# Iselix/kwiiyatta

Measured on AMD Instinct MI355X. Metric: frames/sec end-to-end analyse->align->convert->synth, 48 kHz 5 ms hop, higher is better.
Workload: dtype f64; 1 GPU; config3: 48 kHz source (10 s, T=2001) + target (11 s, T=2201) pairs: CheapTrick+D4C of both, pad with freshly drawn silent spectra, sp2mc, FastDTW(radius 32) align, GMM(64 comp, D=144)+MLPG convert, mc2sp, WORLD synthesis; pairs_per_gpu=32, streams_per_gpu=4, GPU_MAX_HW_QUEUES=4, launch=the whole step is one captured HIP graph, gmm_model_prepared=once per converter (the per-mixture matrices depend on the GMM only), parallelism=pairs in lockstep x32 per GPU, pair-per-GPU x1, no collective

## Files before the change

### kwiiyatta_amd/csrc/kwy_d4c.hip

```cpp
#include <math.h>

#include <vector>

#include "kwy_internal.hpp"

#define D4C_SAFE 0.000000000001
#define D4C_FLOOR_F0 47.0
#define D4C_FREQ_INTERVAL 3000.0
#define D4C_UPPER_LIMIT 15000.0
#define D4C_MAX_BANDS 8

enum { D4C_HANNING = 1, D4C_BLACKMAN = 2 };

__device__ __forceinline__ double d4c_window(int type, int i, int half, double ratio, int fs, double cf0) {
  const double c1 = kwy_cos_pi_range(KWY_PI * ((2.0 * (i - half) / ratio) / fs) * cf0);
  return type == D4C_HANNING ? 0.5 * c1 + 0.5 : 0.42 + 0.5 * c1 + 0.08 * (2.0 * c1 * c1 - 1.0);
}

struct d4c_window_walk {
  double c, s, cd, sd;
  __device__ __forceinline__ d4c_window_walk(int i0, int step, int half, double ratio, int fs, double cf0) {
    kwy_sincos_pi_range(KWY_PI * ((2.0 * (i0 - half) / ratio) / fs) * cf0, &s, &c);
    sincos(KWY_PI * ((2.0 * step / ratio) / fs) * cf0, &sd, &cd);
  }
// ... 316 lines not shown
__device__ inline void d4c_subtract_smoothed(double *io, double *S, double *tot, double width, int fs, int N, int kmax) {
  const int H = N / 2;
  int boundary = (int)(width * N / fs) + 1;
  if (boundary > H / 2) boundary = H / 2;
  const int L = min(H + boundary * 2 + 1, kmax + boundary * 2 + 4);
  kwy_block_cumsum_of<NT, D4C_SMOOTH_CHUNK>([&](int i) {
    double m;
    if (i < boundary) m = io[boundary - i];
    else if (i < H + boundary) m = io[i - boundary];
    else m = io[H - (i - (H + boundary))];
    return m * fs / N;
  }, S, L, tot);
  const double origin = -(boundary - 0.5) * fs / N;
  const double inv_dfi = (double)N / fs, inv_width = 1.0 / width;
  const d4c_taps taps = d4c_smoothing_taps(origin, inv_dfi, width);
  for (int k = threadIdx.x; k <= min(H, kmax); k += NT) io[k] = io[k] - d4c_smoothed_bin(S, L, taps, k) * inv_width;
  __syncthreads();
}

template <int NT, int RK>
__device__ inline void d4c_linear_smoothing_regs(const double *in, double (&outv)[RK], double *S, double *tot,
                                                 double width, int fs, int N) {
  const int H = N / 2;
  int boundary = (int)(width * N / fs) + 1;
  if (boundary > H / 2) boundary = H / 2;
  const int L = H + boundary * 2 + 1;
  kwy_block_cumsum_of<NT, D4C_SMOOTH_CHUNK>([&](int i) {
    double m;
    if (i < boundary) m = in[boundary - i];
    else if (i < H + boundary) m = in[i - boundary];
    else m = in[H - (i - (H + boundary))];
    return m * fs / N;
  }, S, L, tot);
  const double origin = -(boundary - 0.5) * fs / N;
  const double inv_dfi = (double)N / fs, inv_width = 1.0 / width;
  const d4c_taps taps = d4c_smoothing_taps(origin, inv_dfi, width);
#pragma unroll
  for (int r = 0; r < RK; ++r) {
    const int k = threadIdx.x + NT * r;
    outv[r] = 0.0;
    if (k <= H) outv[r] = fmax(d4c_smoothed_bin(S, L, taps, k) * inv_width, 0.0);
  }
  __syncthreads();
}

__device__ __forceinline__ kwy_c d4c_opaque(kwy_c v) {
  asm volatile("" : "+v"(v.x), "+v"(v.y));
  return v;
}

template <int LOG2N>
struct d4c_nt { static constexpr int value = LOG2N >= 13 ? 512 : 256; };
template <int LOG2N>
static constexpr size_t d4c_body_lds() {
  constexpr int N = 1 << LOG2N, H = N / 2, NT = d4c_nt<LOG2N>::value;
  return sizeof(double) * (NT + 16 + D4C_MAX_BANDS + 2) + sizeof(uint32_t) * KWY_EBASE_WORDS +
         (LOG2N >= 12 ? 0 : 8192) + sizeof(double) * ((H + 2) + (2 * H + 2) + 2) +
         ((sizeof(uint32_t) * KWY_SELECT_WORDS(NT) > sizeof(double) * (2 * H + 4))
              ? sizeof(uint32_t) * KWY_SELECT_WORDS(NT) - sizeof(double) * (2 * H + 4) : 0);
}

template <int LOG2N>
__global__ __launch_bounds__(d4c_nt<LOG2N>::value, LOG2N >= 13 ? 1 : 3) void k_d4c_body(
    d4c_batch batch, d4c_params p, kwy_randn_src rs,
    const uint4 *__restrict__ poly, const kwy_c *__restrict__ twH, const kwy_c *__restrict__ twN,
    long long *__restrict__ dbg) {
  constexpr int N = 1 << LOG2N, H = N / 2;
  constexpr int NT = d4c_nt<LOG2N>::value;
  constexpr int E = N / NT;
  constexpr int RK = (H + 1 + NT - 1) / NT;
  constexpr int HEX = 16 * NT / N;
  static_assert(HEX >= 1, "workgroup narrower than N/16");
#define D4C_STAMP(n) do { if (dbg && threadIdx.x == 0 && blockIdx.x == (unsigned)dbg[63]) dbg[n] = clock64(); } while (0)
  extern __shared__ double smem[];
  double *tot = smem;
  double *red = tot + NT;
  double *coarse = red + 16;
  uint32_t *e = (uint32_t *)(coarse + D4C_MAX_BANDS + 2);
  double *jt_own = (double *)(e + KWY_EBASE_WORDS);
  double *A0 = jt_own + (LOG2N >= 12 ? 0 : 1024);
  kwy_c *B = (kwy_c *)(A0 + (H + 2));
  double *Bd = (double *)B;
  double *P = A0, *Dv = A0;
  double *S = Bd;
  uint4 *jtab = (uint4 *)((LOG2N >= 12) ? A0 : jt_own);

  const int tid = threadIdx.x;
  const int utt = batch.find(blockIdx.x);
  const int64_t frame = (int)blockIdx.x - batch.start[utt];
  const double *__restrict__ x = batch.u[utt].x;
  const int x_length = batch.u[utt].x_length;
  const uint64_t *__restrict__ offs3 = batch.u[utt].offs3;
  const uint64_t *__restrict__ draws_before = batch.u[utt].offs_lt + batch.u[utt].T;
  double *__restrict__ dvbuf = batch.u[utt].dvbuf;
  const double f0v = kwy_uniform(batch.u[utt].f0[frame]);
  double *o = batch.u[utt].out + frame * p.K;
  if (f0v == 0.0 || kwy_uniform(batch.u[utt].ap0[frame]) <= p.threshold) {
    for (int k = tid; k < p.K; k += NT) o[k] = 1.0 - D4C_SAFE;
    return;
  }
  const double cf0 = kwy_uniform(f0v > D4C_FLOOR_F0 ? f0v : D4C_FLOOR_F0);
  const double pos = kwy_uniform(batch.u[utt].tpos[frame]);

  D4C_STAMP(0);
  kwy_c tw4[4];
  kwy_fft_thread_twiddles<LOG2N - 1, NT>(twH, tw4);
  const kwy_c twb = twN[tid];
  const uint64_t dbase = *draws_before;
  const uint64_t dpos0 = dbase + offs3[3 * frame], dpos1 = dbase + offs3[3 * frame + 1], dpos2 = dbase + offs3[3 * frame + 2];
  const bool cache = dpos2 + (uint64_t)(2 * kwy_matlab_round(4.0 * p.fs / cf0 / 2.0) + 1) <= rs.n;

  D4C_STAMP(1);
  constexpr int RP = (H / 2 + NT - 1) / NT;
  double cen_lo[RP], cen_hi[RP];
  double *mid = coarse;
  {
    double av[E];
    for (int which = 0; which < 2; ++which) {
      const int tid = kwy_tid_opaque();
      double cpos = which == 0 ? pos - 0.25 / cf0 : pos + 0.25 / cf0;
      d4c_frame_window<N, NT>(x, x_length, p, cf0, cpos, D4C_BLACKMAN, which == 0 ? dpos0 : dpos1, rs, poly, e, jtab, Bd, true, red, av,
                              A0, cache ? 1 + which : 0);
      __syncthreads();
      if (!(tid & 1)) {
#pragma unroll
        for (int r = 0; r < E; ++r) { const int i = tid + NT * r; Bd[i] = av[r]; Bd[i + 1] = av[r] * (i + 1.0); }
      }
      __syncthreads();
      D4C_STAMP(2 + which * 2);
      kwy_fft_inplace_w<LOG2N - 1, NT, false>(B, tw4);
      kwy_c Ek[RP], Eh[RP];
#pragma unroll
      for (int r = 0; r < RP; ++r) {
        const int pp = tid + NT * r;
        Ek[r] = Eh[r] = kwy_c{0.0, 0.0};
        if (pp < H / 2) { Ek[r] = B[pp]; Eh[r] = B[(H - pp) & (H - 1)]; }
      }
      if (tid == 0) { mid[0] = B[H / 2].x; mid[1] = B[H / 2].y; }
      __syncthreads();
      if (tid & 1) {
#pragma unroll
        for (int r = 0; r < E; ++r) { const int i = tid + NT * r; Bd[i - 1] = av[r]; Bd[i] = av[r] * (i + 1.0); }
      }
      __syncthreads();
      kwy_fft_inplace_w<LOG2N - 1, NT, false>(B, tw4);
#pragma unroll
      for (int r = 0; r < RP; ++r) {
        const int pp = tid + NT * r;
        if (pp < H / 2) {
          const kwy_c w = kwy_tw_hex(d4c_opaque(twb), HEX * r);
          const kwy_c Ok = B[pp], Oh = B[(H - pp) & (H - 1)];
          const kwy_c t = cmulf(w, Ok);
          const kwy_c u = cmulf(kwy_c{-w.x, w.y}, Oh);
          const kwy_c zp = cadd(Ek[r], t), zhp = csub(Ek[r], t);
          const kwy_c zq = cadd(Eh[r], u), znp = csub(Eh[r], u);
          const double lo = 2.0 * __builtin_fma(zp.x, znp.y, zp.y * znp.x);
          const double hi = 2.0 * __builtin_fma(zq.x, zhp.y, zq.y * zhp.x);
          cen_lo[r] = which == 0 ? lo : cen_lo[r] + lo;
          cen_hi[r] = which == 0 ? hi : cen_hi[r] + hi;
        }
      }
      if (tid == 0) {
        const kwy_c Em = {mid[0], mid[1]}, Om = B[H / 2];
        const kwy_c t = {Om.y, -Om.x};
        const kwy_c za = cadd(Em, t), zb = csub(Em, t);
        const double v = 2.0 * __builtin_fma(za.x, zb.y, za.y * zb.x);
        mid[2] = which == 0 ? v : mid[2] + v;
      }
      __syncthreads();
      D4C_STAMP(3 + which * 2);
    }

    D4C_STAMP(6);
    d4c_frame_window<N, NT>(x, x_length, p, cf0, pos, D4C_HANNING, dpos2, rs, poly, e, jtab, Bd, false, red, av, A0, cache ? 2 : 0);
#pragma unroll
    for (int r = 0; r < E; ++r) Bd[tid + NT * r] = av[r];
    __syncthreads();
  }
  D4C_STAMP(7);
  kwy_fft_inplace_w<LOG2N - 1, NT, false>(B, tw4);
  D4C_STAMP(8);
  double pv[RK];
  {
    constexpr int Q = (H / 2) / NT;
    static_assert(RK == 2 * Q + 1, "pairs per thread");
#pragma unroll
    for (int q = 0; q < Q; ++q)
      kwy_rfft_pair_power2_w<LOG2N - 1>(B, tid + NT * q, kwy_tw_hex(d4c_opaque(twb), HEX * q), &pv[2 * q], &pv[2 * q + 1]);
    pv[2 * Q] = 0.0;
    if (tid == 0) {
      double pm;
      kwy_rfft_pair_power2_w<LOG2N - 1>(B, H / 2, kwy_c{0.0, -1.0}, &pv[2 * Q], &pm);
    }
    __syncthreads();
#pragma unroll
    for (int q = 0; q < Q; ++q) {
      const int k = tid + NT * q;
      P[k] = pv[2 * q];
      P[H - k] = pv[2 * q + 1];
    }
    if (tid == 0) P[H / 2] = pv[2 * Q];
  }
  __syncthreads();
  d4c_dc_correction<NT>(P, S, cf0, p.fs, N);
  d4c_linear_smoothing_regs<NT, RK>(P, pv, S, tot, cf0, p.fs, N);

  D4C_STAMP(9);
#pragma unroll
  for (int r = 0; r < RP; ++r) {
    const int pp = tid + NT * r;
    if (pp < H / 2) { Dv[pp] = cen_lo[r]; Dv[H - pp] = cen_hi[r]; }
  }
  if (tid == 0) Dv[H / 2] = mid[2];
  __syncthreads();
  d4c_dc_correction<NT>(Dv, S, cf0, p.fs, N);
#pragma unroll
  for (int r = 0; r < RK; ++r)
    if (tid + NT * r <= H) Dv[tid + NT * r] = Dv[tid + NT * r] / pv[r];
  __syncthreads();
  const int kdv = p.dv_len - 1;
  d4c_linear_smoothing<NT>(Dv, Dv, S, tot, cf0 / 2.0, p.fs, N, kdv + 2 * ((int)(cf0 * N / p.fs) + 1) + 4);
  d4c_subtract_smoothed<NT>(Dv, S, tot, cf0, p.fs, N, kdv);

  D4C_STAMP(10);
  {
    double *dv = dvbuf + (size_t)frame * p.dv_stride;
    for (int k = tid; k < p.dv_len; k += NT) dv[k] = Dv[k];
  }
  D4C_STAMP(15);
#undef D4C_STAMP
}

template <int LOG2N>
static constexpr size_t d4c_bands_lds() {
  constexpr int N = 1 << LOG2N, H = N / 2, NT = d4c_nt<LOG2N>::value;
  return sizeof(double) * (16 + D4C_MAX_BANDS + 2 + 2 * NT) + sizeof(double) * ((2 * H + 2) + 2) +
         ((sizeof(uint32_t) * KWY_SELECT_WORDS(NT) > sizeof(double) * (2 * H + 4))
              ? sizeof(uint32_t) * KWY_SELECT_WORDS(NT) - sizeof(double) * (2 * H + 4) : 0);
}

template <int LOG2N, bool SPARSE>
__global__ __launch_bounds__(d4c_nt<LOG2N>::value, LOG2N >= 13 ? 2 : 4) void k_d4c_bands(
    d4c_batch batch, d4c_params p, const kwy_c *__restrict__ twH,
    const kwy_c *__restrict__ twN, const double *__restrict__ nuttall, long long *__restrict__ dbg) {
  constexpr int N = 1 << LOG2N, H = N / 2;
  constexpr int NT = d4c_nt<LOG2N>::value;
  constexpr int E = N / NT;
  constexpr int RK = (H + 1 + NT - 1) / NT;
  constexpr int HEX = 16 * NT / N;
#define D4C_STAMP(n) do { if (dbg && threadIdx.x == 0 && blockIdx.x == (unsigned)dbg[63]) dbg[n] = clock64(); } while (0)
  extern __shared__ double smem[];
  double *red = smem;
  double *coarse = red + 16;
  double *wns = coarse + D4C_MAX_BANDS + 2;
  kwy_c *B = (kwy_c *)(wns + 2 * NT);
  double *Bd = (double *)B;
  uint32_t *hist = (uint32_t *)B;

  const int tid = threadIdx.x;
  const int utt = batch.find(blockIdx.x);
  const int64_t frame = (int)blockIdx.x - batch.start[utt];
  const double *__restrict__ dvbuf = batch.u[utt].dvbuf;
  double *__restrict__ out = batch.u[utt].out;
  const double f0v = kwy_uniform(batch.u[utt].f0[frame]);
  if (f0v == 0.0 || kwy_uniform(batch.u[utt].ap0[frame]) <= p.threshold) return;
  const double cf0 = kwy_uniform(f0v > D4C_FLOOR_F0 ? f0v : D4C_FLOOR_F0);
  const double *Dv = dvbuf + (size_t)frame * p.dv_stride;
  D4C_STAMP(16);

  const int boundary = __builtin_amdgcn_readfirstlane(kwy_matlab_round(N * 8.0 / p.window_length));
  const int half_window_length = p.window_length / 2;
  constexpr bool sparse = SPARSE;
  double ns0 = 0.0, ns1 = 0.0, ns2 = 0.0, nutr[4] = {0.0, 0.0, 0.0, 0.0};
  if constexpr (sparse) {
    if (2 * tid < p.window_length) ns0 = nuttall[2 * tid];
    if (2 * tid + 1 < p.window_length) ns1 = nuttall[2 * tid + 1];
    wns[2 * tid] = ns0; wns[2 * tid + 1] = ns1;
  } else {
#pragma unroll
    for (int r = 0; r < 4; ++r)
      if (tid + NT * r < p.window_length) nutr[r] = nuttall[tid + NT * r];
  }
  const bool mine0 = sparse && tid < H / 8 && 2 * tid < p.window_length;
  const bool mine1 = sparse && tid < H / 8 && 2 * tid + 1 < p.window_length;
  const double *Dfirst = Dv + ((int)(D4C_FREQ_INTERVAL * N / p.fs) - half_window_length);
  double nx0 = (mine0 && p.nbands > 0) ? Dfirst[2 * tid] : 0.0;
  double nx1 = (mine1 && p.nbands > 0) ? Dfirst[2 * tid + 1] : 0.0;
  for (int b = 0; b < p.nbands; ++b) {
    const int tid = kwy_tid_opaque();
    kwy_c tw4[4];
    kwy_fft_thread_twiddles<LOG2N - 1, NT>(twH + (tid - (int)threadIdx.x), tw4);
    const kwy_c twb = twN[tid];
    const double *Dc = Dv + ((int)(D4C_FREQ_INTERVAL * (b + 1) * N / p.fs) - half_window_length);
    const double c0 = nx0, c1 = nx1;
    if (b == 1) D4C_STAMP(17);
    {
      const double *Dn = Dv + ((int)(D4C_FREQ_INTERVAL * (b + 2) * N / p.fs) - half_window_length);
      const bool more = b + 1 < p.nbands;
      nx0 = (mine0 && more) ? Dn[2 * tid] : 0.0;
      nx1 = (mine1 && more) ? Dn[2 * tid + 1] : 0.0;
    }
    if constexpr (sparse) {
      kwy_c a0 = {c0 * wns[2 * tid], c1 * wns[2 * tid + 1]}, a1 = {0.0, 0.0};
      if (tid == 0 && 2 * (H / 8) < p.window_length) a1.x = Dc[2 * (H / 8)] * nuttall[2 * (H / 8)];
      kwy_fft_pass8_first_sparse_core<LOG2N - 1, NT, false>(B, kwy_tw_reg{tw4[0]}, a0, a1);
      kwy_fft_inplace_rest_w<LOG2N - 1, NT, false>(B, tw4);
      if (b == 1) D4C_STAMP(18);
    } else {
#pragma unroll
      for (int r = 0; r < E; ++r) {
        const int j = tid + NT * r;
        Bd[j] = (r < 4 && j < p.window_length) ? Dc[j] * nutr[r < 4 ? r : 0] : 0.0;
      }
      __syncthreads();
      kwy_fft_inplace_w<LOG2N - 1, NT, false>(B, tw4);
    }
    unsigned long long key[RK];
    constexpr int Q = (H / 2) / NT;
    static_assert(RK == 2 * Q + 1, "pairs per thread");
#pragma unroll
    for (int q = 0; q < Q; ++q) {
      double pk, pm;
      kwy_rfft_pair_power2_w<LOG2N - 1>(B, tid + NT * q, kwy_tw_hex(d4c_opaque(twb), HEX * q), &pk, &pm);
      key[2 * q] = (unsigned long long)__double_as_longlong(pk);
      key[2 * q + 1] = (unsigned long long)__double_as_longlong(pm);
    }
    key[2 * Q] = ~0ull;
    if (tid == 0) {
      double pk, pm;
      kwy_rfft_pair_power2_w<LOG2N - 1>(B, H / 2, kwy_c{0.0, -1.0}, &pk, &pm);
      key[2 * Q] = (unsigned long long)__double_as_longlong(pk);
    }
    __syncthreads();
    if (b == 1) D4C_STAMP(19);
    double nsmall, nall;
    kwy_block_smallest_sum<RK, NT>(key, H + 1, H - boundary, hist, red, &nsmall, &nall);
    if (b == 1) D4C_STAMP(20);
    if (dbg && tid == 0 && blockIdx.x == (unsigned)dbg[63])
      for (int q = 0; q < 12; ++q) dbg[24 + 12 * (b & 1) + q] = hist[2 * KWY_SELECT_BINS + q];
    if (tid == 0) {
      double cv = 10 * log10(nsmall / nall);
      cv = cv + (cf0 - 100) / 50.0;
      coarse[b + 1] = cv < 0.0 ? cv : 0.0;
    }
    __syncthreads();
  }
  D4C_STAMP(21);
  if (tid == 0) {
    coarse[0] = -60.0;
    coarse[p.nbands + 1] = -D4C_SAFE;
  }
  __syncthreads();
  double *o = out + frame * p.K;
  const int nn = p.nbands + 2;
  for (int k = tid; k < p.K; k += NT) {
    double xi = (double)k * p.fs / p.fft_size;
    int seg = min((int)(xi / D4C_FREQ_INTERVAL) + 1, p.nbands + 1);
    if (seg < 1) seg = 1;
    if (seg > nn - 1) seg = nn - 1;
    double xa = (seg - 1 <= p.nbands) ? (seg - 1) * D4C_FREQ_INTERVAL : p.fs / 2.0;
    double xb = (seg <= p.nbands) ? seg * D4C_FREQ_INTERVAL : p.fs / 2.0;
    double sfrac = (xi - xa) / (xb - xa);
    double v = coarse[seg - 1] + sfrac * (coarse[seg] - coarse[seg - 1]);
    o[k] = exp10(v / 20.0);
  }
  D4C_STAMP(22);
#undef D4C_STAMP
}

template <int LOG2N>
static int launch_lt(kwy_ctx *ctx, const d4c_batch &b, int fs) {
  constexpr int N = 1 << LOG2N, H = N / 2;
  const kwy_c *twH, *twN;
  const uint4 *poly;
  KWY_TRY(kwy_get_twiddles(ctx, LOG2N - 1, &twH));
  KWY_TRY(kwy_get_twiddles(ctx, LOG2N, &twN));
  constexpr int NT = d4c_nt<LOG2N>::value;
  KWY_TRY(kwy_get_poly_multi(ctx, N / NT, NT, &poly));
  size_t lds = sizeof(kwy_c) * (H + 1) + sizeof(double) * 8 + sizeof(uint32_t) * KWY_EBASE_WORDS;
  KWY_HIP(hipFuncSetAttribute((const void *)k_d4c_lovetrain<LOG2N, NT>,
                              hipFuncAttributeMaxDynamicSharedMemorySize, (int)lds));
  KWY_PROF(ctx, "k_d4c_lovetrain", hipLaunchKernelGGL((k_d4c_lovetrain<LOG2N, NT>), dim3((unsigned)b.start[b.n]), dim3(NT), lds,
                     ctx->stream, b, fs, kwy_randn(ctx), poly, twH, twN));
  KWY_HIP(hipGetLastError());
  return KWY_OK;
}
// ... 208 lines not shown
```

### kwiiyatta_amd/csrc/kwy_device.hpp

```cpp
#pragma once

#include <hip/hip_runtime.h>
#include <stdint.h>

#define KWY_THREADS 256
#define KWY_WAVES (KWY_THREADS / 64)
#define KWY_PI 3.1415926535897932384

struct kwy_rng {
  uint32_t x, y, z, w;
};

__device__ __forceinline__ void kwy_rng_seed(kwy_rng &r) {
  r.x = 123456789u; r.y = 362436069u; r.z = 521288629u; r.w = 88675123u;
}

__device__ __forceinline__ uint32_t kwy_rng_step(kwy_rng &r) {
  uint32_t t = r.x ^ (r.x << 11);
  r.x = r.y; r.y = r.z; r.z = r.w;
  r.w = (r.w ^ (r.w >> 19)) ^ (t ^ (t >> 8));
  return r.w;
}

__device__ __forceinline__ uint32_t kwy_rng_randn_raw(kwy_rng &r) {
  uint32_t tmp = kwy_rng_step(r) >> 4;
#pragma unroll
  for (int i = 0; i < 11; ++i) tmp += kwy_rng_step(r) >> 4;
  return tmp;
}
__device__ __forceinline__ double kwy_rng_randn(kwy_rng &r) {
  return kwy_rng_randn_raw(r) / 268435456.0 - 6.0;
}

__device__ __forceinline__ uint32_t kwy_wave_xor_u32(uint32_t v) {
  v ^= (uint32_t)__builtin_amdgcn_update_dpp(0, (int)v, 0x111, 0xf, 0xf, true);
  v ^= (uint32_t)__builtin_amdgcn_update_dpp(0, (int)v, 0x112, 0xf, 0xf, true);
  v ^= (uint32_t)__builtin_amdgcn_update_dpp(0, (int)v, 0x114, 0xf, 0xf, true);
  v ^= (uint32_t)__builtin_amdgcn_update_dpp(0, (int)v, 0x118, 0xf, 0xf, true);
  return (uint32_t)__builtin_amdgcn_readlane((int)v, 15) ^ (uint32_t)__builtin_amdgcn_readlane((int)v, 31) ^
         (uint32_t)__builtin_amdgcn_readlane((int)v, 47) ^ (uint32_t)__builtin_amdgcn_readlane((int)v, 63);
}

__device__ inline void kwy_wave_jump(uint32_t (&s)[4], uint64_t steps, const uint4 *__restrict__ pow2) {
  const int lane = threadIdx.x & 63;
  for (int k = 0; steps != 0; ++k, steps >>= 1) {
    if (!(steps & 1)) continue;
    const uint32_t wlo = lane < 32 ? s[0] : s[1];
    const uint32_t whi = lane < 32 ? s[2] : s[3];
    uint32_t o0 = 0, o1 = 0, o2 = 0, o3 = 0;
    uint32_t m = 0u - ((wlo >> (lane & 31)) & 1u);
    uint4 c = pow2[k * 128 + lane];
    o0 ^= c.x & m; o1 ^= c.y & m; o2 ^= c.z & m; o3 ^= c.w & m;
    m = 0u - ((whi >> (lane & 31)) & 1u);
    c = pow2[k * 128 + 64 + lane];
    o0 ^= c.x & m; o1 ^= c.y & m; o2 ^= c.z & m; o3 ^= c.w & m;
    s[0] = kwy_wave_xor_u32(o0); s[1] = kwy_wave_xor_u32(o1);
    s[2] = kwy_wave_xor_u32(o2); s[3] = kwy_wave_xor_u32(o3);
  }
}

#define KWY_EBASE_WORDS 132
__device__ inline void kwy_rng_ebase(kwy_rng s, uint32_t *e) {
  e[0] = s.x; e[1] = s.y; e[2] = s.z; e[3] = s.w;
  for (int i = 4; i < 131; ++i) e[i] = kwy_rng_step(s);
  e[131] = 0;
}

__device__ __forceinline__ void kwy_rng_combine_word(kwy_rng &r, const uint32_t *e, uint32_t bits,
                                                      uint32_t &w0, uint32_t &w1, uint32_t &w2) {
#pragma unroll 8
  for (int b = 0; b < 32; ++b) {
    uint32_t w3 = e[b + 3];
    uint32_t m = 0u - ((bits >> b) & 1u);
    r.x ^= w0 & m; r.y ^= w1 & m; r.z ^= w2 & m; r.w ^= w3 & m;
    w0 = w1; w1 = w2; w2 = w3;
  }
}

__device__ __forceinline__ kwy_rng kwy_rng_combine(const uint32_t *e, uint4 c) {
  kwy_rng r = {0, 0, 0, 0};
  uint32_t w0 = e[0], w1 = e[1], w2 = e[2];
  kwy_rng_combine_word(r, e, c.x, w0, w1, w2);
  kwy_rng_combine_word(r, e + 32, c.y, w0, w1, w2);
  kwy_rng_combine_word(r, e + 64, c.z, w0, w1, w2);
  kwy_rng_combine_word(r, e + 96, c.w, w0, w1, w2);
  return r;
}

__device__ __forceinline__ void kwy_lds_barrier() {
  asm volatile("s_waitcnt lgkmcnt(0)\n\ts_barrier" ::: "memory");
}

struct kwy_randn_src {
  const uint32_t *tab;
  uint64_t n;
  const uint4 *pow2;
};
// ... 718 lines not shown
  if constexpr (LOG2H == 12) kwy_fft_pass8<LOG2H, 9, NT, INV>(z, tw);
  if constexpr (LOG2H == 11) kwy_fft_tail<LOG2H, 2, NT, INV>(z);
  if constexpr (LOG2H == 10) kwy_fft_tail<LOG2H, 1, NT, INV>(z);
}

template <int LOG2H, int TAIL, int NT, bool INV>
__device__ __forceinline__ void kwy_fft_tail(kwy_c *z) {
  constexpr int H = 1 << LOG2H, R = 1 << TAIL, Q = H / R;
  constexpr int IT = (Q + NT - 1) / NT;
  kwy_c a[IT][R];
  const int tid = kwy_tid_opaque();
#pragma unroll
  for (int it = 0; it < IT; ++it) {
    const int j = tid + it * NT;
    if (j < Q) {
#pragma unroll
      for (int m = 0; m < R; ++m) a[it][m] = z[j + m * Q];
      if constexpr (TAIL == 2) {
        kwy_c apc = cadd(a[it][0], a[it][2]), amc = csub(a[it][0], a[it][2]);
        kwy_c bpd = cadd(a[it][1], a[it][3]), jb = kwy_rot90<INV>(csub(a[it][1], a[it][3]));
        a[it][0] = cadd(apc, bpd); a[it][1] = cadd(amc, jb);
        a[it][2] = csub(apc, bpd); a[it][3] = csub(amc, jb);
      } else {
        kwy_c s0 = cadd(a[it][0], a[it][1]), s1 = csub(a[it][0], a[it][1]);
        a[it][0] = s0; a[it][1] = s1;
      }
#pragma unroll
      for (int m = 0; m < R; ++m) z[j + m * Q] = a[it][m];
    }
  }
  __syncthreads();
}

template <int LOG2H, int NT, bool INV>
__device__ inline void kwy_fft_inplace(kwy_c *z, const kwy_c *__restrict__ tw) {
  static_assert(LOG2H >= 8 && LOG2H <= 12, "unsupported in-place FFT length");
  kwy_fft_pass8<LOG2H, 0, NT, INV>(z, tw);
  kwy_fft_pass8<LOG2H, 3, NT, INV>(z, tw);
  if constexpr (LOG2H >= 9) kwy_fft_pass8<LOG2H, 6, NT, INV>(z, tw);
  if constexpr (LOG2H == 12) kwy_fft_pass8<LOG2H, 9, NT, INV>(z, tw);
  if constexpr (LOG2H % 3 != 0) kwy_fft_tail<LOG2H, LOG2H % 3, NT, INV>(z);
}

template <int LOG2H, int NT>
__device__ __forceinline__ void kwy_fft_thread_twiddles(const kwy_c *__restrict__ twH, kwy_c (&w)[4]) {
  static_assert((1 << LOG2H) / 8 <= NT, "one butterfly per thread and pass");
  const int j = threadIdx.x;
#pragma unroll
  for (int p = 0; p < 4; ++p) {
    const int ps = (j >> (3 * p)) << (3 * p);
    w[p] = (3 * p + 3 < LOG2H + 0 && ps < (1 << LOG2H) / 8) ? twH[ps] : kwy_c{1.0, 0.0};
  }
}
template <int LOG2H, int NT, bool INV>
__device__ inline void kwy_fft_inplace_rest_w(kwy_c *z, const kwy_c (&w)[4]) {
  kwy_fft_pass8_core<LOG2H, 3, NT, INV>(z, kwy_tw_reg{w[1]});
  if constexpr (LOG2H >= 9) kwy_fft_pass8_core<LOG2H, 6, NT, INV>(z, kwy_tw_reg{w[2]});
  if constexpr (LOG2H == 12) kwy_fft_pass8_core<LOG2H, 9, NT, INV>(z, kwy_tw_reg{w[3]});
  if constexpr (LOG2H % 3 != 0) kwy_fft_tail<LOG2H, LOG2H % 3, NT, INV>(z);
}
template <int LOG2H, int NT, bool INV>
__device__ inline void kwy_fft_inplace_w(kwy_c *z, const kwy_c (&w)[4]) {
  static_assert(LOG2H >= 8 && LOG2H <= 12, "unsupported in-place FFT length");
  kwy_fft_pass8_core<LOG2H, 0, NT, INV>(z, kwy_tw_reg{w[0]});
  kwy_fft_inplace_rest_w<LOG2H, NT, INV>(z, w);
}

__device__ __forceinline__ kwy_c kwy_tw_hex(kwy_c b, int idx16) {
  if (!(idx16 & 1)) return kwy_tw_octant(b, idx16 >> 1);
  const double c1 = 0.92387953251128675613, s1 = 0.38268343236508977173;
  double wr, wi;
  switch (idx16 & 15) {
    case 1: wr = c1; wi = -s1; break;
    case 3: wr = s1; wi = -c1; break;
    case 5: wr = -s1; wi = -c1; break;
    case 7: wr = -c1; wi = -s1; break;
    case 9: wr = -c1; wi = s1; break;
    case 11: wr = -s1; wi = c1; break;
    case 13: wr = s1; wi = c1; break;
    default: wr = c1; wi = s1; break;
  }
  return {__builtin_fma(b.x, wr, -(b.y * wi)), __builtin_fma(b.x, wi, b.y * wr)};
}

template <int LOG2H, int NT>
__device__ inline void kwy_rfft_inplace(kwy_c *z, const kwy_c *__restrict__ tw, kwy_c twb,
                                   const kwy_c *__restrict__ twN = nullptr) {
  constexpr int H = 1 << LOG2H, N = 2 * H;
  constexpr int OCT = 8 * NT / N;
  kwy_fft_inplace<LOG2H, NT, false>(z, tw);
  const int tid = kwy_tid_opaque();
#pragma unroll
  for (int r = 0; r * NT <= H / 2; ++r) {
    const int k = tid + NT * r;
    if (k > H / 2) continue;
    if (k == 0) {
      const kwy_c z0 = z[0];
      z[0] = {z0.x + z0.y, 0.0};
      z[H] = {z0.x - z0.y, 0.0};
    } else {
      const kwy_c w = (OCT >= 1) ? kwy_tw_octant(twb, OCT * r) : twN[k];
      const kwy_c A = z[k], Bc = z[H - k];
      const double er = 0.5 * (A.x + Bc.x), ei = 0.5 * (A.y - Bc.y);
      const double dr = 0.5 * (A.x - Bc.x), di = 0.5 * (A.y + Bc.y);
      const double orr = di, oi = -dr;
      const double pr = __builtin_fma(orr, w.x, -(oi * w.y)), pi = __builtin_fma(orr, w.y, oi * w.x);
      z[k] = {er + pr, ei + pi};
      if (k != H - k) z[H - k] = {er - pr, -(ei - pi)};
    }
  }
  __syncthreads();
}

template <int LOG2H, int NT>
__device__ inline void kwy_irfft_inplace(kwy_c *z, const kwy_c *__restrict__ tw, kwy_c twb,
                                   const kwy_c *__restrict__ twN = nullptr) {
  constexpr int H = 1 << LOG2H, N = 2 * H;
  constexpr int OCT = 8 * NT / N;
// ... 10 lines not shown
      const kwy_c w = (OCT >= 1) ? kwy_tw_octant(twb, OCT * r) : twN[k];
      const kwy_c A = z[k], Bc = z[H - k];
      const double er = A.x + Bc.x, ei = A.y - Bc.y;
      const double dr = A.x - Bc.x, di = A.y + Bc.y;
      const double wr = w.x, wi = -w.y;
      const double orr = __builtin_fma(dr, wr, -(di * wi)), oi = __builtin_fma(dr, wi, di * wr);
      z[k] = {er - oi, ei + orr};
      if (k != H - k) z[H - k] = {er + oi, -(ei - orr)};
    }
  }
  __syncthreads();
  kwy_fft_inplace<LOG2H, NT, true>(z, tw);
}

template <int LOG2H>
__device__ __forceinline__ kwy_c kwy_rfft_bin_w(const kwy_c *z, int k, kwy_c w) {
  constexpr int H = 1 << LOG2H;
  if (k == 0) return {z[0].x + z[0].y, 0.0};
  if (k == H) return {z[0].x - z[0].y, 0.0};
  const kwy_c A = z[k];
  const kwy_c B = {z[H - k].x, -z[H - k].y};
  const double er = 0.5 * (A.x + B.x), ei = 0.5 * (A.y + B.y);
  const double dr = 0.5 * (A.x - B.x), di = 0.5 * (A.y - B.y);
  const double orr = di, oi = -dr;
  return {er + (orr * w.x - oi * w.y), ei + (orr * w.y + oi * w.x)};
}
template <int LOG2H>
__device__ __forceinline__ kwy_c kwy_rfft_bin2_w(const kwy_c *z, int k, kwy_c w) {
  constexpr int H = 1 << LOG2H;
  if (k == 0) return {2.0 * (z[0].x + z[0].y), 0.0};
  if (k == H) return {2.0 * (z[0].x - z[0].y), 0.0};
  const kwy_c A = z[k];
  const kwy_c B = {z[H - k].x, -z[H - k].y};
  const double er = A.x + B.x, ei = A.y + B.y;
  const double dr = A.x - B.x, di = A.y - B.y;
  return {__builtin_fma(dr, w.y, __builtin_fma(di, w.x, er)), __builtin_fma(-dr, w.x, __builtin_fma(di, w.y, ei))};
}
template <int LOG2H>
__device__ __forceinline__ void kwy_rfft_pair_power2_w(const kwy_c *z, int k, kwy_c w, double *pk, double *pm) {
  constexpr int H = 1 << LOG2H;
  if (k == 0) {
    const double a = 2.0 * (z[0].x + z[0].y), b = 2.0 * (z[0].x - z[0].y);
    *pk = a * a; *pm = b * b;
    return;
  }
  const kwy_c A = z[k], Bz = z[H - k];
  const double er = A.x + Bz.x, ei = A.y - Bz.y;
  const double dr = A.x - Bz.x, di = A.y + Bz.y;
  const double pr = __builtin_fma(dr, w.y, di * w.x), pi = __builtin_fma(-dr, w.x, di * w.y);
  const double xr = er + pr, xi = ei + pi, yr = er - pr, yi = ei - pi;
  *pk = __builtin_fma(xr, xr, xi * xi);
  *pm = __builtin_fma(yr, yr, yi * yi);
}
template <int LOG2H>
__device__ __forceinline__ kwy_c kwy_rfft_bin(const kwy_c *z, int k, const kwy_c *__restrict__ twN) {
  return kwy_rfft_bin_w<LOG2H>(z, k, twN[k & ((2 << LOG2H) - 1)]);
}

__device__ __forceinline__ int kwy_matlab_round(double x) {
  return x > 0 ? (int)(x + 0.5) : (int)(x - 0.5);
}
```

### kwiiyatta_amd/csrc/kwy_selftest.h

```cpp
#ifndef KWY_SELFTEST_H_
#define KWY_SELFTEST_H_
#ifdef __cplusplus
extern "C" {
#endif
int kwy_debug_smallest_sum_dev(void *stream, const double *values, int problems, int n, int m, double *out);
int kwy_debug_devmath_dev(void *stream, const double *x, int n, double *log_out, double *sin_out, double *cos_out);
#ifdef __cplusplus
}
#endif
#endif
```

### kwiiyatta_amd/csrc/selftest/kwy_selftest.hip

```cpp
#include <hip/hip_runtime.h>

#include <stdint.h>

#include "../kwy_device.hpp"
#include "../kwy_selftest.h"

#define D4C_NT 256

__global__ __launch_bounds__(D4C_NT) void k_select_selftest(const double *__restrict__ v, int n, int m,
                                                           double *__restrict__ out) {
  constexpr int RK = 9;
  __shared__ __attribute__((aligned(16))) uint32_t hist[KWY_SELECT_WORDS(D4C_NT)];
  __shared__ double red[2 * D4C_NT / 64];
  const int tid = threadIdx.x;
  const double *x = v + (size_t)blockIdx.x * n;
  unsigned long long key[RK];
#pragma unroll
  for (int r = 0; r < RK; ++r) {
    const int k = tid + D4C_NT * r;
    key[r] = k < n ? (unsigned long long)__double_as_longlong(x[k]) : ~0ull;
  }
  double s_small, s_all;
  kwy_block_smallest_sum<RK, D4C_NT>(key, n, m, hist, red, &s_small, &s_all);
  if (tid == 0) { out[2 * blockIdx.x] = s_small; out[2 * blockIdx.x + 1] = s_all; }
}

extern "C" int kwy_debug_smallest_sum_dev(void *stream, const double *values, int problems, int n, int m,
                                          double *out) {
  if (!values || !out || problems <= 0 || n <= 0 || n > 9 * D4C_NT || m <= 0 || m > n) return -1;
  hipLaunchKernelGGL(k_select_selftest, dim3(problems), dim3(D4C_NT), 0, (hipStream_t)stream, values, n, m, out);
  return hipGetLastError() == hipSuccess ? 0 : -2;
}

__global__ void k_devmath_selftest(const double *__restrict__ x, int n, double *__restrict__ lg, double *__restrict__ sn,
                                   double *__restrict__ cs) {
  const int i = blockIdx.x * blockDim.x + threadIdx.x;
  if (i >= n) return;
  lg[i] = kwy_log(x[i]);
  kwy_sincos_medium(x[i], &sn[i], &cs[i]);
}

extern "C" int kwy_debug_devmath_dev(void *stream, const double *x, int n, double *log_out, double *sin_out,
                                     double *cos_out) {
  if (!x || !log_out || !sin_out || !cos_out || n <= 0) return -1;
  hipLaunchKernelGGL(k_devmath_selftest, dim3((n + 255) / 256), dim3(256), 0, (hipStream_t)stream, x, n, log_out,
                     sin_out, cos_out);
  return hipGetLastError() == hipSuccess ? 0 : -2;
}
```

Before: 2.601 million frames/s.

## Fuse radix-4 FFT tail into register drain for 4096-point D4C transforms

```diff
diff --git a/kwiiyatta_amd/csrc/kwy_d4c.hip b/kwiiyatta_amd/csrc/kwy_d4c.hip
--- a/kwiiyatta_amd/csrc/kwy_d4c.hip
+++ b/kwiiyatta_amd/csrc/kwy_d4c.hip
@@ -392,6 +392,9 @@
 template <int LOG2N>
 struct d4c_nt { static constexpr int value = LOG2N >= 13 ? 512 : 256; };
 template <int LOG2N>
+struct d4c_drain { static constexpr bool value = LOG2N == 12; };
+#define D4C_DRAIN_TWC(twN, NT, tid) (twN)[((NT) - (tid)) & ((NT) - 1)]
+template <int LOG2N>
 static constexpr size_t d4c_body_lds() {
   constexpr int N = 1 << LOG2N, H = N / 2, NT = d4c_nt<LOG2N>::value;
   return sizeof(double) * (NT + 16 + D4C_MAX_BANDS + 2) + sizeof(uint32_t) * KWY_EBASE_WORDS +
@@ -411,6 +414,7 @@
   constexpr int RK = (H + 1 + NT - 1) / NT;
   constexpr int HEX = 16 * NT / N;
   static_assert(HEX >= 1, "workgroup narrower than N/16");
+  constexpr bool DRAIN = d4c_drain<LOG2N>::value;
 #define D4C_STAMP(n) do { if (dbg && threadIdx.x == 0 && blockIdx.x == (unsigned)dbg[63]) dbg[n] = clock64(); } while (0)
   extern __shared__ double smem[];
   double *tot = smem;
@@ -445,6 +449,8 @@
   D4C_STAMP(0);
   kwy_c tw4[4];
   kwy_fft_thread_twiddles<LOG2N - 1, NT>(twH, tw4);
+#define D4C_BODY_TW4() do { if constexpr (DRAIN) { const int ot = kwy_tid_opaque(); \
+    kwy_fft_thread_twiddles<LOG2N - 1, NT>(twH + (ot - (int)threadIdx.x), tw4); } } while (0)
   const kwy_c twb = twN[tid];
   const uint64_t dbase = *draws_before;
   const uint64_t dpos0 = dbase + offs3[3 * frame], dpos1 = dbase + offs3[3 * frame + 1], dpos2 = dbase + offs3[3 * frame + 2];
@@ -468,28 +474,51 @@
       }
       __syncthreads();
       D4C_STAMP(2 + which * 2);
-      kwy_fft_inplace_w<LOG2N - 1, NT, false>(B, tw4);
+      D4C_BODY_TW4();
+      kwy_fft_inplace_w<LOG2N - 1, NT, false, !DRAIN>(B, tw4);
       kwy_c Ek[RP], Eh[RP];
+      if constexpr (DRAIN) {
+        static_assert(RP == 4, "four pairs per thread");
+        kwy_c Em;
+        kwy_fft_tail4_drain<LOG2N - 1, NT, false>(B, Ek, Eh, Em);
+        if (tid == 0) { mid[0] = Em.x; mid[1] = Em.y; }
+      } else {
+#pragma unroll
+        for (int r = 0; r < RP; ++r) {
+          const int pp = tid + NT * r;
+          Ek[r] = Eh[r] = kwy_c{0.0, 0.0};
+          if (pp < H / 2) { Ek[r] = B[pp]; Eh[r] = B[(H - pp) & (H - 1)]; }
+        }
+        if (tid == 0) { mid[0] = B[H / 2].x; mid[1] = B[H / 2].y; }
+      }
+      __syncthreads();
+      if (tid & 1) {
+#pragma unroll
+        for (int r = 0; r < E; ++r) { const int i = tid + NT * r; Bd[i - 1] = av[r]; Bd[i] = av[r] * (i + 1.0); }
+      }
+      __syncthreads();
+      D4C_BODY_TW4();
+      kwy_fft_inplace_w<LOG2N - 1, NT, false, !DRAIN>(B, tw4);
+      kwy_c Od[DRAIN ? 4 : 1], Odh[DRAIN ? 4 : 1], twa = {0.0, 0.0}, twc = {0.0, 0.0};
+      if constexpr (DRAIN) {
+        kwy_c Om;
+        kwy_fft_tail4_drain<LOG2N - 1, NT, false>(B, Od, Odh, Om);
+        if (tid == 0) { mid[3] = Om.x; mid[4] = Om.y; }
+        twa = twN[tid];
+        twc = D4C_DRAIN_TWC(twN, NT, tid);
+      }
 #pragma unroll
       for (int r = 0; r < RP; ++r) {
         const int pp = tid + NT * r;
-        Ek[r] = Eh[r] = kwy_c{0.0, 0.0};
-        if (pp < H / 2) { Ek[r] = B[pp]; Eh[r] = B[(H - pp) & (H - 1)]; }
-      }
-      if (tid == 0) { mid[0] = B[H / 2].x; mid[1] = B[H / 2].y; }
-      __syncthreads();
-      if (tid & 1) {
-#pragma unroll
-        for (int r = 0; r < E; ++r) { const int i = tid + NT * r; Bd[i - 1] = av[r]; Bd[i] = av[r] * (i + 1.0); }
-      }
-      __syncthreads();
-      kwy_fft_inplace_w<LOG2N - 1, NT, false>(B, tw4);
-#pragma unroll
-      for (int r = 0; r < RP; ++r) {
-        const int pp = tid + NT * r;
-        if (pp < H / 2) {
-          const kwy_c w = kwy_tw_hex(d4c_opaque(twb), HEX * r);
-          const kwy_c Ok = B[pp], Oh = B[(H - pp) & (H - 1)];
+        if (DRAIN || pp < H / 2) {
+          kwy_c w, Ok, Oh;
+          if constexpr (DRAIN) {
+            w = kwy_drain_tw<LOG2N - 1, NT>(r, twa, twc);
+            Ok = Od[r]; Oh = Odh[r];
+          } else {
+            w = kwy_tw_hex(d4c_opaque(twb), HEX * r);
+            Ok = B[pp]; Oh = B[(H - pp) & (H - 1)];
+          }
           const kwy_c t = cmulf(w, Ok);
           const kwy_c u = cmulf(kwy_c{-w.x, w.y}, Oh);
           const kwy_c zp = cadd(Ek[r], t), zhp = csub(Ek[r], t);
@@ -501,7 +530,7 @@
         }
       }
       if (tid == 0) {
-        const kwy_c Em = {mid[0], mid[1]}, Om = B[H / 2];
+        const kwy_c Em = {mid[0], mid[1]}, Om = DRAIN ? kwy_c{mid[3], mid[4]} : B[H / 2];
         const kwy_c t = {Om.y, -Om.x};
         const kwy_c za = cadd(Em, t), zb = csub(Em, t);
         const double v = 2.0 * __builtin_fma(za.x, zb.y, za.y * zb.x);
@@ -518,10 +547,35 @@
     __syncthreads();
   }
   D4C_STAMP(7);
-  kwy_fft_inplace_w<LOG2N - 1, NT, false>(B, tw4);
+  D4C_BODY_TW4();
+  kwy_fft_inplace_w<LOG2N - 1, NT, false, !DRAIN>(B, tw4);
   D4C_STAMP(8);
   double pv[RK];
-  {
+  if constexpr (DRAIN) {
+    static_assert(RK == 9, "four pairs per thread and the self-paired bin");
+    const int tid = kwy_tid_opaque();
+    kwy_c lo[4], hi[4], md;
+    kwy_fft_tail4_drain<LOG2N - 1, NT, false>(B, lo, hi, md);
+    const kwy_c twa = twN[tid], twc = D4C_DRAIN_TWC(twN, NT, tid);
+#pragma unroll
+    for (int s = 0; s < 4; ++s) {
+      if (s == 0 && tid == 0) kwy_rfft_pair_power2_dc(lo[0], &pv[0], &pv[1]);
+      else kwy_rfft_pair_power2_v(lo[s], hi[s], kwy_drain_tw<LOG2N - 1, NT>(s, twa, twc), &pv[2 * s], &pv[2 * s + 1]);
+    }
+    pv[8] = 0.0;
+    if (tid == 0) {
+      double pm;
+      kwy_rfft_pair_power2_v(md, md, kwy_c{0.0, -1.0}, &pv[8], &pm);
+    }
+    __syncthreads();
+#pragma unroll
+    for (int s = 0; s < 4; ++s) {
+      const int k = kwy_drain_bin<LOG2N - 1>(s, tid);
+      P[k] = pv[2 * s];
+      P[H - k] = pv[2 * s + 1];
+    }
+    if (tid == 0) P[H / 2] = pv[8];
+  } else {
     constexpr int Q = (H / 2) / NT;
     static_assert(RK == 2 * Q + 1, "pairs per thread");
 #pragma unroll
@@ -548,7 +602,7 @@
   D4C_STAMP(9);
 #pragma unroll
   for (int r = 0; r < RP; ++r) {
-    const int pp = tid + NT * r;
+    const int pp = DRAIN ? kwy_drain_bin<LOG2N - 1>(r, tid) : tid + NT * r;
     if (pp < H / 2) { Dv[pp] = cen_lo[r]; Dv[H - pp] = cen_hi[r]; }
   }
   if (tid == 0) Dv[H / 2] = mid[2];
@@ -569,6 +623,7 @@
   }
   D4C_STAMP(15);
 #undef D4C_STAMP
+#undef D4C_BODY_TW4
 }
 
 template <int LOG2N>
@@ -588,6 +643,7 @@
   constexpr int E = N / NT;
   constexpr int RK = (H + 1 + NT - 1) / NT;
   constexpr int HEX = 16 * NT / N;
+  constexpr bool DRAIN = d4c_drain<LOG2N>::value;
 #define D4C_STAMP(n) do { if (dbg && threadIdx.x == 0 && blockIdx.x == (unsigned)dbg[63]) dbg[n] = clock64(); } while (0)
   extern __shared__ double smem[];
   double *red = smem;
@@ -644,7 +700,7 @@
       kwy_c a0 = {c0 * wns[2 * tid], c1 * wns[2 * tid + 1]}, a1 = {0.0, 0.0};
       if (tid == 0 && 2 * (H / 8) < p.window_length) a1.x = Dc[2 * (H / 8)] * nuttall[2 * (H / 8)];
       kwy_fft_pass8_first_sparse_core<LOG2N - 1, NT, false>(B, kwy_tw_reg{tw4[0]}, a0, a1);
-      kwy_fft_inplace_rest_w<LOG2N - 1, NT, false>(B, tw4);
+      kwy_fft_inplace_rest_w<LOG2N - 1, NT, false, !DRAIN>(B, tw4);
       if (b == 1) D4C_STAMP(18);
     } else {
 #pragma unroll
@@ -653,25 +709,56 @@
         Bd[j] = (r < 4 && j < p.window_length) ? Dc[j] * nutr[r < 4 ? r : 0] : 0.0;
       }
       __syncthreads();
-      kwy_fft_inplace_w<LOG2N - 1, NT, false>(B, tw4);
+      kwy_fft_inplace_w<LOG2N - 1, NT, false, !DRAIN>(B, tw4);
     }
     unsigned long long key[RK];
     constexpr int Q = (H / 2) / NT;
     static_assert(RK == 2 * Q + 1, "pairs per thread");
-#pragma unroll
-    for (int q = 0; q < Q; ++q) {
-      double pk, pm;
-      kwy_rfft_pair_power2_w<LOG2N - 1>(B, tid + NT * q, kwy_tw_hex(d4c_opaque(twb), HEX * q), &pk, &pm);
-      key[2 * q] = (unsigned long long)__double_as_longlong(pk);
-      key[2 * q + 1] = (unsigned long long)__double_as_longlong(pm);
-    }
-    key[2 * Q] = ~0ull;
-    if (tid == 0) {
-      double pk, pm;
-      kwy_rfft_pair_power2_w<LOG2N - 1>(B, H / 2, kwy_c{0.0, -1.0}, &pk, &pm);
-      key[2 * Q] = (unsigned long long)__double_as_longlong(pk);
-    }
-    __syncthreads();
+    if constexpr (DRAIN) {
+      static_assert(Q == 4 && sizeof(uint32_t) * KWY_SELECT_WORDS(NT) <= sizeof(kwy_c) * NT, "exchange clear of the histogram");
+      kwy_c lo[4], hi[4], md;
+      kwy_fft_tail4_drain<LOG2N - 1, NT, false>(B, lo, hi, md);
+      const kwy_c twc = D4C_DRAIN_TWC(twN, NT, tid);
+      double pw[8];
+#pragma unroll
+      for (int s = 0; s < 4; ++s) {
+        if (s == 0 && tid == 0) kwy_rfft_pair_power2_dc(lo[0], &pw[0], &pw[1]);
+        else kwy_rfft_pair_power2_v(lo[s], hi[s], kwy_drain_tw<LOG2N - 1, NT>(s, d4c_opaque(twb), twc), &pw[2 * s], &pw[2 * s + 1]);
+      }
+      key[2 * Q] = ~0ull;
+      if (tid == 0) {
+        double pk, pm;
+        kwy_rfft_pair_power2_v(md, md, kwy_c{0.0, -1.0}, &pk, &pm);
+        key[2 * Q] = (unsigned long long)__double_as_longlong(pk);
+      } else {
+        B[2 * NT - tid] = kwy_c{pw[4], pw[5]};
+        B[4 * NT - tid] = kwy_c{pw[6], pw[7]};
+      }
+      __syncthreads();
+      if (tid != 0) {
+        const kwy_c v1 = B[NT + tid], v3 = B[3 * NT + tid];
+        pw[4] = v1.x; pw[5] = v1.y; pw[6] = v3.x; pw[7] = v3.y;
+      }
+      key[0] = (unsigned long long)__double_as_longlong(pw[0]); key[1] = (unsigned long long)__double_as_longlong(pw[1]);
+      key[2] = (unsigned long long)__double_as_longlong(pw[4]); key[3] = (unsigned long long)__double_as_longlong(pw[5]);
+      key[4] = (unsigned long long)__double_as_longlong(pw[2]); key[5] = (unsigned long long)__double_as_longlong(pw[3]);
+      key[6] = (unsigned long long)__double_as_longlong(pw[6]); key[7] = (unsigned long long)__double_as_longlong(pw[7]);
+    } else {
+#pragma unroll
+      for (int q = 0; q < Q; ++q) {
+        double pk, pm;
+        kwy_rfft_pair_power2_w<LOG2N - 1>(B, tid + NT * q, kwy_tw_hex(d4c_opaque(twb), HEX * q), &pk, &pm);
+        key[2 * q] = (unsigned long long)__double_as_longlong(pk);
+        key[2 * q + 1] = (unsigned long long)__double_as_longlong(pm);
+      }
+      key[2 * Q] = ~0ull;
+      if (tid == 0) {
+        double pk, pm;
+        kwy_rfft_pair_power2_w<LOG2N - 1>(B, H / 2, kwy_c{0.0, -1.0}, &pk, &pm);
+        key[2 * Q] = (unsigned long long)__double_as_longlong(pk);
+      }
+      __syncthreads();
+    }
     if (b == 1) D4C_STAMP(19);
     double nsmall, nall;
     kwy_block_smallest_sum<RK, NT>(key, H + 1, H - boundary, hist, red, &nsmall, &nall);
diff --git a/kwiiyatta_amd/csrc/kwy_device.hpp b/kwiiyatta_amd/csrc/kwy_device.hpp
--- a/kwiiyatta_amd/csrc/kwy_device.hpp
+++ b/kwiiyatta_amd/csrc/kwy_device.hpp
@@ -42,7 +42,8 @@
 }
 
 __device__ inline void kwy_wave_jump(uint32_t (&s)[4], uint64_t steps, const uint4 *__restrict__ pow2) {
-  const int lane = threadIdx.x & 63;
+  int lane = threadIdx.x & 63;
+  asm volatile("" : "+v"(lane));
   for (int k = 0; steps != 0; ++k, steps >>= 1) {
     if (!(steps & 1)) continue;
     const uint32_t wlo = lane < 32 ? s[0] : s[1];
@@ -867,18 +868,18 @@
     w[p] = (3 * p + 3 < LOG2H + 0 && ps < (1 << LOG2H) / 8) ? twH[ps] : kwy_c{1.0, 0.0};
   }
 }
-template <int LOG2H, int NT, bool INV>
+template <int LOG2H, int NT, bool INV, bool TAIL = true>
 __device__ inline void kwy_fft_inplace_rest_w(kwy_c *z, const kwy_c (&w)[4]) {
   kwy_fft_pass8_core<LOG2H, 3, NT, INV>(z, kwy_tw_reg{w[1]});
   if constexpr (LOG2H >= 9) kwy_fft_pass8_core<LOG2H, 6, NT, INV>(z, kwy_tw_reg{w[2]});
   if constexpr (LOG2H == 12) kwy_fft_pass8_core<LOG2H, 9, NT, INV>(z, kwy_tw_reg{w[3]});
-  if constexpr (LOG2H % 3 != 0) kwy_fft_tail<LOG2H, LOG2H % 3, NT, INV>(z);
-}
-template <int LOG2H, int NT, bool INV>
+  if constexpr (TAIL && LOG2H % 3 != 0) kwy_fft_tail<LOG2H, LOG2H % 3, NT, INV>(z);
+}
+template <int LOG2H, int NT, bool INV, bool TAIL = true>
 __device__ inline void kwy_fft_inplace_w(kwy_c *z, const kwy_c (&w)[4]) {
   static_assert(LOG2H >= 8 && LOG2H <= 12, "unsupported in-place FFT length");
   kwy_fft_pass8_core<LOG2H, 0, NT, INV>(z, kwy_tw_reg{w[0]});
-  kwy_fft_inplace_rest_w<LOG2H, NT, INV>(z, w);
+  kwy_fft_inplace_rest_w<LOG2H, NT, INV, TAIL>(z, w);
 }
 
 __device__ __forceinline__ kwy_c kwy_tw_hex(kwy_c b, int idx16) {
@@ -995,6 +996,73 @@
   *pk = __builtin_fma(xr, xr, xi * xi);
   *pm = __builtin_fma(yr, yr, yi * yi);
 }
+__device__ __forceinline__ kwy_c kwy_rfft_bin2_v(kwy_c A, kwy_c Bz, kwy_c w) {
+  const kwy_c B = {Bz.x, -Bz.y};
+  const double er = A.x + B.x, ei = A.y + B.y;
+  const double dr = A.x - B.x, di = A.y - B.y;
+  return {__builtin_fma(dr, w.y, __builtin_fma(di, w.x, er)), __builtin_fma(-dr, w.x, __builtin_fma(di, w.y, ei))};
+}
+__device__ __forceinline__ void kwy_rfft_pair_power2_v(kwy_c A, kwy_c Bz, kwy_c w, double *pk, double *pm) {
+  const double er = A.x + Bz.x, ei = A.y - Bz.y;
+  const double dr = A.x - Bz.x, di = A.y + Bz.y;
+  const double pr = __builtin_fma(dr, w.y, di * w.x), pi = __builtin_fma(-dr, w.x, di * w.y);
+  const double xr = er + pr, xi = ei + pi, yr = er - pr, yi = ei - pi;
+  *pk = __builtin_fma(xr, xr, xi * xi);
+  *pm = __builtin_fma(yr, yr, yi * yi);
+}
+__device__ __forceinline__ void kwy_rfft_pair_power2_dc(kwy_c Z0, double *pk, double *pm) {
+  const double a = 2.0 * (Z0.x + Z0.y), b = 2.0 * (Z0.x - Z0.y);
+  *pk = a * a; *pm = b * b;
+}
+
+template <int LOG2H, int NT, bool INV>
+__device__ __forceinline__ void kwy_fft_tail4_drain(const kwy_c *z, kwy_c (&lo)[4], kwy_c (&hi)[4], kwy_c &mid) {
+  constexpr int H = 1 << LOG2H, Q = H / 4;
+  static_assert(LOG2H % 3 == 2 && NT == Q / 2, "radix-4 tail, two butterflies per thread");
+  const int t = kwy_tid_opaque();
+  const int jb = t ? Q - t : Q / 2;
+  kwy_c a[4], b[4];
+#pragma unroll
+  for (int m = 0; m < 4; ++m) { a[m] = z[t + m * Q]; b[m] = z[jb + m * Q]; }
+  {
+    const kwy_c apc = cadd(a[0], a[2]), amc = csub(a[0], a[2]);
+    const kwy_c bpd = cadd(a[1], a[3]), jq = kwy_rot90<INV>(csub(a[1], a[3]));
+    a[0] = cadd(apc, bpd); a[1] = cadd(amc, jq); a[2] = csub(apc, bpd); a[3] = csub(amc, jq);
+  }
+  {
+    const kwy_c apc = cadd(b[0], b[2]), amc = csub(b[0], b[2]);
+    const kwy_c bpd = cadd(b[1], b[3]), jq = kwy_rot90<INV>(csub(b[1], b[3]));
+    b[0] = cadd(apc, bpd); b[1] = cadd(amc, jq); b[2] = csub(apc, bpd); b[3] = csub(amc, jq);
+  }
+  const bool t0 = t == 0;
+  lo[0] = a[0]; hi[0] = t0 ? a[0] : b[3];
+  lo[1] = a[1]; hi[1] = t0 ? a[3] : b[2];
+  lo[2] = b[0]; hi[2] = t0 ? b[3] : a[3];
+  lo[3] = b[1]; hi[3] = t0 ? b[2] : a[2];
+  mid = a[2];
+}
+template <int LOG2H>
+__device__ __forceinline__ int kwy_drain_bin(int s, int t) {
+  constexpr int Q = (1 << LOG2H) / 4;
+  switch (s) {
+    case 0: return t;
+    case 1: return Q + t;
+    case 2: return t ? Q - t : Q / 2;
+    default: return t ? 2 * Q - t : Q + Q / 2;
+  }
+}
+template <int LOG2H, int NT>
+__device__ __forceinline__ kwy_c kwy_drain_tw(int s, kwy_c twa, kwy_c twc) {
+  constexpr int HEX = 16 * NT / (2 << LOG2H);
+  static_assert(HEX >= 1, "workgroup narrower than N/16");
+  switch (s) {
+    case 0: return kwy_tw_hex(twa, 0);
+    case 1: return kwy_tw_hex(twa, 2 * HEX);
+    case 2: return kwy_tw_hex(twc, HEX);
+    default: return kwy_tw_hex(twc, 3 * HEX);
+  }
+}
+
 template <int LOG2H>
 __device__ __forceinline__ kwy_c kwy_rfft_bin(const kwy_c *z, int k, const kwy_c *__restrict__ twN) {
   return kwy_rfft_bin_w<LOG2H>(z, k, twN[k & ((2 << LOG2H) - 1)]);
diff --git a/kwiiyatta_amd/csrc/kwy_selftest.h b/kwiiyatta_amd/csrc/kwy_selftest.h
--- a/kwiiyatta_amd/csrc/kwy_selftest.h
+++ b/kwiiyatta_amd/csrc/kwy_selftest.h
@@ -5,6 +5,7 @@
 #endif
 int kwy_debug_smallest_sum_dev(void *stream, const double *values, int problems, int n, int m, double *out);
 int kwy_debug_devmath_dev(void *stream, const double *x, int n, double *log_out, double *sin_out, double *cos_out);
+int kwy_debug_rfft_paths_dev(void *stream, const double *x, int problems, int log2n, double *out_old, double *out_new);
 #ifdef __cplusplus
 }
 #endif
diff --git a/kwiiyatta_amd/csrc/selftest/kwy_selftest.hip b/kwiiyatta_amd/csrc/selftest/kwy_selftest.hip
--- a/kwiiyatta_amd/csrc/selftest/kwy_selftest.hip
+++ b/kwiiyatta_amd/csrc/selftest/kwy_selftest.hip
@@ -1,6 +1,9 @@
 #include <hip/hip_runtime.h>
 
+#include <math.h>
 #include <stdint.h>
+
+#include <vector>
 
 #include "../kwy_device.hpp"
 #include "../kwy_selftest.h"
@@ -47,3 +50,71 @@
                      sin_out, cos_out);
   return hipGetLastError() == hipSuccess ? 0 : -2;
 }
+
+template <int LOG2N, int NT>
+__global__ __launch_bounds__(NT) void k_rfft_paths_selftest(const double *__restrict__ x, const kwy_c *__restrict__ twH,
+                                                            const kwy_c *__restrict__ twN, kwy_c *__restrict__ out_old,
+                                                            kwy_c *__restrict__ out_new) {
+  constexpr int N = 1 << LOG2N, H = N / 2, HEX = 16 * NT / N;
+  extern __shared__ double smem[];
+  kwy_c *B = (kwy_c *)smem;
+  double *Bd = smem;
+  const int tid = threadIdx.x;
+  const double *row = x + (size_t)blockIdx.x * N;
+  kwy_c *oo = out_old + (size_t)blockIdx.x * (H + 1), *on = out_new + (size_t)blockIdx.x * (H + 1);
+  kwy_c tw4[4];
+  kwy_fft_thread_twiddles<LOG2N - 1, NT>(twH, tw4);
+  for (int i = tid; i < N; i += NT) Bd[i] = row[i];
+  __syncthreads();
+  kwy_fft_inplace_w<LOG2N - 1, NT, false>(B, tw4);
+  for (int r = 0; tid + NT * r <= H; ++r) {
+    const int k = tid + NT * r;
+    const kwy_c w = r < 4 ? kwy_tw_hex(twN[tid], HEX * r) : twN[k];
+    oo[k] = kwy_rfft_bin2_w<LOG2N - 1>(B, k, w);
+  }
+  __syncthreads();
+  for (int i = tid; i < N; i += NT) Bd[i] = row[i];
+  __syncthreads();
+  kwy_fft_inplace_w<LOG2N - 1, NT, false, false>(B, tw4);
+  kwy_c lo[4], hi[4], md;
+  kwy_fft_tail4_drain<LOG2N - 1, NT, false>(B, lo, hi, md);
+  const kwy_c twa = twN[tid], twc = twN[(NT - tid) & (NT - 1)];
+#pragma unroll
+  for (int s = 0; s < 4; ++s) {
+    const int k = kwy_drain_bin<LOG2N - 1>(s, tid);
+    if (k == 0) {
+      on[0] = {2.0 * (lo[0].x + lo[0].y), 0.0};
+      on[H] = {2.0 * (lo[0].x - lo[0].y), 0.0};
+    } else {
+      on[k] = kwy_rfft_bin2_v(lo[s], hi[s], kwy_drain_tw<LOG2N - 1, NT>(s, twa, twc));
+      on[H - k] = kwy_rfft_bin2_v(hi[s], lo[s], twN[H - k]);
+    }
+  }
+  if (tid == 0) on[H / 2] = kwy_rfft_bin2_v(md, md, twN[H / 2]);
+}
+
+extern "C" int kwy_debug_rfft_paths_dev(void *stream, const double *x, int problems, int log2n, double *out_old,
+                                        double *out_new) {
+  if (!x || !out_old || !out_new || problems <= 0) return -1;
+  if (log2n != 12) return -1;
+  constexpr int LOG2N = 12, NT = 256, N = 1 << LOG2N, H = N / 2;
+  std::vector<kwy_c> h(H / 8 + N);
+  for (int k = 0; k < H / 8; ++k) { const double a = -2.0 * KWY_PI * k / H; h[k] = {cos(a), sin(a)}; }
+  for (int k = 0; k < N; ++k) { const double a = -2.0 * KWY_PI * k / N; h[H / 8 + k] = {cos(a), sin(a)}; }
+  kwy_c *tw = nullptr;
+  if (hipMalloc((void **)&tw, sizeof(kwy_c) * h.size()) != hipSuccess) return -2;
+  int rc = 0;
+  if (hipMemcpy(tw, h.data(), sizeof(kwy_c) * h.size(), hipMemcpyHostToDevice) != hipSuccess) rc = -2;
+  if (rc == 0) {
+    const size_t lds = sizeof(kwy_c) * (H + 1);
+    auto kern = k_rfft_paths_selftest<LOG2N, NT>;
+    if (hipFuncSetAttribute((const void *)kern, hipFuncAttributeMaxDynamicSharedMemorySize, (int)lds) != hipSuccess) rc = -2;
+    if (rc == 0) {
+      hipLaunchKernelGGL(kern, dim3(problems), dim3(NT), lds, (hipStream_t)stream, x, tw, tw + H / 8, (kwy_c *)out_old,
+                         (kwy_c *)out_new);
+      if (hipGetLastError() != hipSuccess || hipStreamSynchronize((hipStream_t)stream) != hipSuccess) rc = -2;
+    }
+  }
+  hipFree(tw);
+  return rc;
+}
```

After: 2.661 million frames/s, median of 6. 1.02x the previous value.
